# vincekurtz/quadruped_drake

Measured on NVIDIA B200. Metric: whole-body QP control steps/sec, higher is better.
Workload: dtype f64

## Files before the change

### quadruped_drake_b200/csrc/wbc_device.cuh

```cuda
#pragma once
#include <stdint.h>
#include <math.h>
#include <stddef.h>
#include <type_traits>
#include "wbc.h"

#ifndef WBC_DEV
#define WBC_DEV __device__ __forceinline__
#endif
#ifndef WBC_FULL
#define WBC_FULL 0xffffffffu
#endif

namespace wbc {

constexpr int NF = 13;
constexpr int YS = 15;
constexpr int YROWS = 32;
constexpr int AR = 6;
constexpr int AC = 32;
constexpr double RANKDEF_SINVOL = 2e-3;

struct Derived {
  double clf_p[3][3];
// ... 341 lines not shown
    s.vf[leg][j] = comp(vfoot, j);
  }
  if (lane == 0 && !BIAS_ONLY) {
    s.task[7] = R0.c0.x; s.task[8] = R0.c0.y; s.task[9] = R0.c0.z;
    s.task[10] = R0.c1.x; s.task[11] = R0.c1.y; s.task[12] = R0.c1.z;
    s.task[13] = R0.c2.x; s.task[14] = R0.c2.y; s.task[15] = R0.c2.z;
  }
  __syncwarp();
}

#ifdef __CUDACC__
__device__ __noinline__
#else
static
#endif
void dynamics_pc_pass(WarpSmem& s, const wbc_model& md, int lane, int& status, const double* vel_int, double* bias_out, bool bias,
                      double* taug_out = nullptr) {
  dynamics_phase<DYN_PC>(s, md, lane, status, taug_out, vel_int, bias_out, bias);
}

struct BodyTask { double rpy[3], rpyd[3]; double N[3][3]; };
WBC_DEV void body_task(const WarpSmem& s, int lane, int& status, BodyTask& t) {
  const double r00 = s.task[7], r10 = s.task[8], r20 = s.task[9], r21 = s.task[12], r22 = s.task[15];
  const double cp = sqrt(r00 * r00 + r10 * r10);
  const int m = lane % 3;
  double num = m == 0 ? r21 : (m == 1 ? -r20 : r10);
  double den = m == 0 ? r22 : (m == 1 ? cp : r00);
  double ang = atan2(num, den);
  t.rpy[0] = shfl(ang, 0); t.rpy[1] = shfl(ang, 1); t.rpy[2] = shfl(ang, 2);
  double cy, sy;
  const double icp = cp < 1e-6 ? 0.0 : frcp(cp);
  if (cp < 1e-6) { status |= WBC_ST_GIMBAL; cy = 1.0; sy = 0.0; }
  else { cy = r00 * icp; sy = r10 * icp; }
  const double sp = -r20;
  t.N[0][0] = cy * cp; t.N[0][1] = -sy; t.N[0][2] = 0.0;
  t.N[1][0] = sy * cp; t.N[1][1] = cy;  t.N[1][2] = 0.0;
  t.N[2][0] = -sp;     t.N[2][1] = 0.0; t.N[2][2] = 1.0;
  const double wx = s.v[0], wy = s.v[1], wz = s.v[2];
  t.rpyd[0] = (cy * wx + sy * wy) * icp;
  t.rpyd[1] = -sy * wx + cy * wy;
  t.rpyd[2] = wz + sp * t.rpyd[0];
}

WBC_DEV double skew_ent(V3 r, int i, int c) {
  if (i == c) return 0.0;
  const double m = comp(r, 3 - i - c);
  return ((i + 1) % 3 == c) ? -m : m;
}
WBC_DEV int stance_slot(unsigned cmask, int k) {
  return ((cmask >> k) & 1) ? __popc(cmask & ((1u << k) - 1)) : -1;
}
WBC_DEV int stance_foot(unsigned cmask, int slot) {
  int k = 0, cnt = 0;
#pragma unroll
  for (int kk = 0; kk < 4; ++kk) { if ((cmask >> kk) & 1) { if (cnt == slot) k = kk; ++cnt; } }
  return k;
}

WBC_DEV void build_base_system(WarpSmem& s, int lane, unsigned cmask, double kd, int& status) {
  bool bad = false;
  if (lane < 12) {
    const int k = lane / 3, i = lane % 3;
    if ((cmask >> k) & 1) {
      const int i1 = (i + 1) % 3, i2 = (i + 2) % 3;
      const V3 ci = mk(s.L[k][0][i], s.L[k][1][i], s.L[k][2][i]);
      const V3 c1 = mk(s.L[k][0][i1], s.L[k][1][i1], s.L[k][2][i1]);
      const V3 c2 = mk(s.L[k][0][i2], s.L[k][1][i2], s.L[k][2][i2]);
      const V3 cx = cross(c1, c2);
      const double det = dot(ci, cx);
      const double vol2 = dot(ci, ci) * dot(c1, c1) * dot(c2, c2);
      bad = !(det * det > RANKDEF_SINVOL * RANKDEF_SINVOL * vol2);
      const V3 li = frcp(bad ? 1.0 : det) * cx;
      const V3 rh = ld3(s.rho[k]);
      const V3 lxr = cross(rh, li);
      s.AK[k][i][0] = lxr.x; s.AK[k][i][1] = lxr.y; s.AK[k][i][2] = lxr.z;
      s.AK[k][i][3] = li.x; s.AK[k][i][4] = li.y; s.AK[k][i][5] = li.z;
      const V3 r = mk(-s.Jdv[k][0] - kd * s.vf[k][0], -s.Jdv[k][1] - kd * s.vf[k][1], -s.Jdv[k][2] - kd * s.vf[k][2]);
      s.AK[k][i][6] = dot(li, r);
    }
  }
  if (__any_sync(WBC_FULL, bad)) status |= WBC_ST_RANKDEF;
  __syncwarp();
  const int c = lane;
  double col[AR];
#pragma unroll
  for (int r = 0; r < AR; ++r) col[r] = 0.0;
  if (c < 6 || c == 31) {
    const int cc = c < 6 ? c : 6;
#pragma unroll
    for (int r = 0; r < 6; ++r) col[r] = c < 6 ? s.Mb[c][r] : -s.hb[r];
#pragma unroll
    for (int k = 0; k < 4; ++k) {
      if (!((cmask >> k) & 1)) continue;
#pragma unroll
      for (int a = 0; a < 3; ++a) {
        const double ak = s.AK[k][a][cc];
#pragma unroll
        for (int r = 0; r < 6; ++r) col[r] = fma(-s.Mb[6 + 3 * k + a][r], ak, col[r]);
      }
    }
  } else if (c < 18) {
    const int k = (c - 6) / 3, i = (c - 6) % 3;
    if ((cmask >> k) & 1) {
      const V3 rh = ld3(s.rho[k]);
#pragma unroll
      for (int r = 0; r < 3; ++r) { col[r] = skew_ent(rh, i, r); col[3 + r] = (r == i) ? -1.0 : 0.0; }
    } else {
#pragma unroll
      for (int r = 0; r < 6; ++r) col[r] = s.Mb[c][r];
    }
  }
#pragma unroll
  for (int r = 0; r < AR; ++r) s.A[r][c] = col[r];
  __syncwarp();
}

WBC_DEV unsigned gauss_jordan(WarpSmem& s, int lane, int m, int n, int& status, unsigned long long& rowmap) {
  unsigned used = 0;
  rowmap = 0ull;
  for (int r = 0; r < m; ++r) {
    const double arc0 = s.A[r][lane];
    const bool eligible = lane < n && !((used >> lane) & 1);
    int pcol;
    const double best = warp_max_lane(eligible ? fabs(arc0) : 0.0, pcol);
    if (!(best > 1e-9)) {
      status |= WBC_ST_RANKDEF;
      continue;
    }
    const double piv = shfl(arc0, pcol);
    const double arc = arc0 * frcp(piv);
    if (lane != pcol) {
#pragma unroll
      for (int i = 0; i < AR; ++i) {
        if (i < m) {
          const double f = s.A[i][pcol];
          s.A[i][lane] = fma(-f, arc, s.A[i][lane]);
        }
      }
      s.A[r][lane] = arc;
    }
    rowmap |= (unsigned long long)(r + 1) << (3 * pcol);
    used |= 1u << pcol;
    __syncwarp();
  }
  return used;
}

WBC_DEV double zent(const WarpSmem& s, int lane, int var, unsigned long long rowmap) {
  const int r = (int)((rowmap >> (3 * var)) & 7ull) - 1;
  const double a = s.A[r >= 0 ? r : 0][lane];
  return r >= 0 ? (lane == 31 ? a : -a) : (var == lane ? 1.0 : 0.0);
}

struct TriPairs { int i[3], k[3]; };
template <int N> WBC_DEV TriPairs tri_pairs(int lane) {
  TriPairs t;
#pragma unroll
  for (int h = 0; h < 3; ++h) {
    const int e = lane + 32 * h;
    int ii = 0;
#pragma unroll
    for (int c = 1; c < N; ++c) ii += (c * (c + 1) / 2 <= e) ? 1 : 0;
    t.i[h] = e < N * (N + 1) / 2 ? ii : -1;
    t.k[h] = e - ii * (ii + 1) / 2;
  }
  return t;
}

template <int N, class SM> WBC_DEV void reduced_hessian(SM& s, int lane, int nf, bool tau_rows, bool extra, const TriPairs& tp) {
  s.y[lane] = s.cw[lane] * (s.Y[lane][NF] - s.ct[lane]);
  const double wb = s.cw[0], wl0 = s.cw[6], wl1 = s.cw[9], wl2 = s.cw[12], wl3 = s.cw[15];
#pragma unroll
  for (int h = 0; h < 3; ++h) {
    const int i = tp.i[h], k = tp.k[h];
    if (i < 0) continue;
    const double* yi = &s.Y[0][i];
    const double* yk = &s.Y[0][k];
    auto term = [&](int r) { return yi[r * YS] * yk[r * YS]; };
    auto leg = [&](int r) { return fma(yi[(r + 2) * YS], yk[(r + 2) * YS], fma(yi[(r + 1) * YS], yk[(r + 1) * YS], term(r))); };
    const double b0 = fma(yi[2 * YS], yk[2 * YS], fma(yi[1 * YS], yk[1 * YS], term(0)));
    const double b1 = fma(yi[5 * YS], yk[5 * YS], fma(yi[4 * YS], yk[4 * YS], term(3)));
    double acc = wb * (b0 + b1);
    acc = fma(wl0, leg(6), acc); acc = fma(wl1, leg(9), acc); acc = fma(wl2, leg(12), acc); acc = fma(wl3, leg(15), acc);
    if (tau_rows) {
      double t0 = 0.0, t1 = 0.0;
#pragma unroll
      for (int r = 18; r < 30; r += 2) { t0 = fma(yi[r * YS], yk[r * YS], t0); t1 = fma(yi[(r + 1) * YS], yk[(r + 1) * YS], t1); }
      acc = fma(s.cw[18], t0 + t1, acc);
    }
    if (extra) acc = fma(s.cw[30] * yi[30 * YS], yk[30 * YS], fma(s.cw[31] * yi[31 * YS], yk[31 * YS], acc));
    if (i >= nf) acc = (i == k) ? 1.0 : 0.0;
    s.H[i][k] = acc;
  }
  __syncwarp();
}

template <int N, class SM> WBC_DEV void cholesky_factor(SM& s, int lane, int& status, const TriPairs& tp) {
  for (int j = 0; j < N; ++j) {
    const double dj = s.H[j][j];
    if (!(dj > 1e-300)) { status |= WBC_ST_NOTPD; }
    const double rd = frcp(dj > 1e-300 ? dj : 1.0);
#pragma unroll
    for (int h = 0; h < 3; ++h) {
      const int i = tp.i[h], k = tp.k[h];
      if (i >= 0 && k > j) s.H[i][k] = fma(-s.H[i][j] * rd, s.H[k][j], s.H[i][k]);
    }
    __syncwarp();
  }
  if (lane < N) { const double dk = s.H[lane][lane]; s.d[lane] = frsqrt(dk > 1e-300 ? dk : 1.0); }
  __syncwarp();
#pragma unroll
  for (int h = 0; h < 3; ++h) {
    const int i = tp.i[h], k = tp.k[h];
    if (i >= 0) s.H[i][k] *= s.d[k];
  }
  __syncwarp();
}
struct Ineq { int ra, rb; double ca, cb, bound; };
struct IneqSet {
  unsigned cmask; double mu; int nfric; int nextra; int ntl; const double* effort;
  double extra_bound[2];
};
WBC_DEV Ineq get_ineq(const IneqSet& S, int i) {
  Ineq q; q.ra = q.rb = 0; q.ca = q.cb = 0.0; q.bound = 0.0;
  if (i < S.nfric) {
    int sl = i >> 2, t = i & 3, k = 0, cnt = 0;
#pragma unroll
    for (int kk = 0; kk < 4; ++kk) { if ((S.cmask >> kk) & 1) { if (cnt == sl) k = kk; ++cnt; } }
    q.ra = 6 + 3 * k + (t >> 1); q.ca = (t & 1) ? -1.0 : 1.0;
    q.rb = 6 + 3 * k + 2; q.cb = -S.mu; q.bound = 0.0;
  } else if (i < S.nfric + S.nextra) {
    const int e = i - S.nfric;
    q.ra = 30 + e; q.ca = 1.0; q.bound = S.extra_bound[e];
  } else {
    const int e = i - S.nfric - S.nextra;
    const int k = e % 12;
    q.ra = 18 + k; q.ca = e < 12 ? 1.0 : -1.0; q.bound = S.effort[k];
  }
  return q;
}

template <int N, class SM> WBC_DEV double tri_fwd_lane(const SM& s, int lane, double rhs) {
  const bool row = lane < N;
  const int li = row ? lane : N - 1;
  const double dinv = s.d[li];
  double acc = row ? rhs : 0.0, bl = 0.0;
#pragma unroll
  for (int j = 0; j < N; ++j) {
    const double bj = shfl(acc * dinv, j);
    if (lane == j) bl = bj;
    else if (lane > j) acc = fma(-s.H[li][j], bj, acc);
  }
  return bl;
}
template <int N, class SM> WBC_DEV double tri_bwd_lane(const SM& s, int lane, double rhs) {
  const bool row = lane < N;
  const int li = row ? lane : N - 1;
  const double dinv = s.d[li];
  double acc = row ? rhs : 0.0, xl = 0.0;
#pragma unroll
  for (int j = N - 1; j >= 0; --j) {
    const double xj = shfl(acc * dinv, j);
    if (lane == j) xl = xj;
    else if (lane < j) acc = fma(-s.H[j][li], xj, acc);
  }
  return xl;
}

template <int N, class SM> WBC_DEV int gi_solve_ws(SM& s, int lane, const IneqSet& S, int max_iter, int& status, int& q_out,
                                                  double& minslack, const double* Yg) {
  const int mi = S.nfric + S.nextra + S.ntl;
  const bool row = lane < N;
  const int li = row ? lane : N - 1;
  const Ineq c0 = get_ineq(S, lane < mi ? lane : 0);
  const bool have0 = lane < mi;
  double* Wl = &s.Y[lane][0];
  double yl;
  {
    double w[N];
#pragma unroll
    for (int k = 0; k < N; ++k) {
      double acc = Wl[k];
#pragma unroll
      for (int j = 0; j < k; ++j) acc = fma(-w[j], s.H[k][j], acc);
      w[k] = acc * s.d[k];
    }
#pragma unroll
    for (int k = 0; k < N; ++k) Wl[k] = w[k];
    __syncwarp();
    {
      const double* wc = &s.Y[0][li];
      double b0 = 0.0, b1 = 0.0;
#pragma unroll
      for (int r = 0; r < 18; r += 2) { b0 = fma(wc[r * YS], s.y[r], b0); b1 = fma(wc[(r + 1) * YS], s.y[r + 1], b1); }
      if (s.cw[18] != 0.0) {
#pragma unroll
        for (int r = 18; r < 30; r += 2) { b0 = fma(wc[r * YS], s.y[r], b0); b1 = fma(wc[(r + 1) * YS], s.y[r + 1], b1); }
      }
      b0 = fma(wc[30 * YS], s.y[30], b0); b1 = fma(wc[31 * YS], s.y[31], b1);
      if (row) s.dm[lane] = b0 + b1;
    }
    __syncwarp();
    double ya = Wl[NF], ya1 = 0.0;
#pragma unroll
    for (int k = 0; k < N; ++k) { if (k & 1) ya1 = fma(-w[k], s.dm[k], ya1); else ya = fma(-w[k], s.dm[k], ya); }
    yl = ya + ya1;
    __syncwarp();
    s.y[lane] = yl;
  }
  __syncwarp();
  double ddl0 = 0.0, ddl1 = 0.0;
  {
    const double* wa = &s.Y[c0.ra][0];
    const double* wb = &s.Y[c0.rb][0];
#pragma unroll
    for (int k = 0; k < N; ++k) { const double t = fma(c0.ca, wa[k], c0.cb * wb[k]); ddl0 = fma(t, t, ddl0); }
    if (mi > 32) {
      const Ineq c1 = get_ineq(S, lane + 32 < mi ? lane + 32 : 0);
      const double* va = &s.Y[c1.ra][0];
      const double* vb = &s.Y[c1.rb][0];
#pragma unroll
      for (int k = 0; k < N; ++k) { const double t = fma(c1.ca, va[k], c1.cb * vb[k]); ddl1 = fma(t, t, ddl1); }
    }
  }
  double* const Ril = ri_rows(s) + li * NF;
  {
    double* r0 = ri_rows(s);
    for (int e = lane; e < NF * NF; e += 32) r0[e] = 0.0;
  }
  __syncwarp();
  int q = 0, iters = 0;
  unsigned long long activemask = 0ull;
  double ul = 0.0;
  int actl = 0;
  minslack = 0.0;
  double violl = 0.0;
  auto select = [&](bool& any, int& p_out, int& wl) {
    double viol = 0.0; int who = lane;
    if (have0 && !((activemask >> lane) & 1ull)) {
      const double ta = c0.ca * s.y[c0.ra], tb = c0.cb * s.y[c0.rb];
      const double sl = c0.bound - ta - tb;
      if (sl < -1e-10 * (1.0 + fabs(c0.bound) + fabs(ta) + fabs(tb))) viol = -sl;
    }
    if (mi > 32) {
      const Ineq c1 = get_ineq(S, lane + 32 < mi ? lane + 32 : 0);
      if (lane + 32 < mi && !((activemask >> (lane + 32)) & 1ull)) {
        const double ta = c1.ca * s.y[c1.ra], tb = c1.cb * s.y[c1.rb];
        const double sl = c1.bound - ta - tb;
        if (sl < -1e-10 * (1.0 + fabs(c1.bound) + fabs(ta) + fabs(tb)) && -sl > viol) { viol = -sl; who = lane + 32; }
      }
    }
    violl = viol;
    wl = warp_argmax_hi(viol, any);
    p_out = (mi > 32) ? shfl(who, wl) : wl;
  };
  bool any; int p, wlane;
  select(any, p, wlane);
  for (;;) {
    if (!any) break;
    Ineq cp;
    if (p < 32) {
      const int rr = shfl(c0.ra | (c0.rb << 8), p);
      cp.ra = rr & 0xff; cp.rb = rr >> 8;
      cp.ca = shfl(c0.ca, p); cp.cb = shfl(c0.cb, p); cp.bound = shfl(c0.bound, p);
    } else {
      cp = get_ineq(S, p);
    }
    const double nca = -cp.ca, ncb = -cp.cb;
    double up = 0.0;
    bool fail = false;
    const double dd = (p < 32) ? shfl(ddl0, p & 31) : shfl(ddl1, p & 31);
    for (;;) {
      if (++iters > max_iter) { status |= WBC_ST_MAXITER; fail = true; break; }
      const double dself = fma(nca, s.Y[cp.ra][li], ncb * s.Y[cp.rb][li]);
      if (row) s.dm[lane] = dself;
      __syncwarp();
      double zn = 0.0, zn1 = 0.0, wd = 0.0, wd1 = 0.0;
      switch (q) {
#define WBC_ACC(K)                                                                                   \
        case K:                                                                                      \
          if (K < N) {                                                                               \
            const double dk_ = s.dm[K < N ? K : 0];                                                  \
            if (K & 1) { zn1 = fma(dk_, dk_, zn1); wd1 = fma(Wl[K < N ? K : 0], dk_, wd1); }         \
            else { zn = fma(dk_, dk_, zn); wd = fma(Wl[K < N ? K : 0], dk_, wd); }                   \
          }
        WBC_ACC(0) WBC_ACC(1) WBC_ACC(2) WBC_ACC(3) WBC_ACC(4) WBC_ACC(5) WBC_ACC(6) WBC_ACC(7) WBC_ACC(8) WBC_ACC(9) WBC_ACC(10)
        WBC_ACC(11) WBC_ACC(12)
#undef WBC_ACC
        default: break;
      }
      double rk = 0.0, rk1 = 0.0;
      switch (q) {
#define WBC_RI(K)                                                                                    \
        case K + 1:                                                                                  \
          if (K < N) {                                                                               \
            if (K & 1) rk1 = fma(Ril[K < N ? K : 0], s.dm[K < N ? K : 0], rk1);                      \
            else rk = fma(Ril[K < N ? K : 0], s.dm[K < N ? K : 0], rk);                              \
          }
        WBC_RI(12) WBC_RI(11) WBC_RI(10) WBC_RI(9) WBC_RI(8) WBC_RI(7) WBC_RI(6) WBC_RI(5) WBC_RI(4) WBC_RI(3) WBC_RI(2) WBC_RI(1)
        WBC_RI(0)
#undef WBC_RI
        default: break;
      }
      zn += zn1; wd += wd1; rk += rk1;
      const int qc = q < N ? q : N - 1;
      const double dq = s.dm[qc], wq = Wl[qc];
      const double sp = cp.bound - cp.ca * s.y[cp.ra] - cp.cb * s.y[cp.rb];
      const bool zok = zn > 1e-14 * fmax(dd, 1e-300);
      const double zs = zok ? zn : 1.0;
      const double izn = frcp(zs);
      const double rs = frsqrt(zs);
      const double nrm = zs * rs;
      const double alpha = dq > 0.0 ? -nrm : nrm;
      const double hv = fma(-dq, alpha, zs);
      const double ihv = frcp(hv);
      int l;
      const double t1 = warp_min_lane((lane < q && rk > 0.0) ? fmax(ul * frcp(rk), 0.0) + 0.0 : INFINITY, l);
      const double t2 = zok ? -sp * izn : INFINITY;
      const double t = fmin(t1, t2);
      if (!(t < INFINITY)) { status |= WBC_ST_INFEASIBLE; fail = true; break; }
      const bool dual_only = !(t2 < INFINITY);
      if (lane < q) ul -= t * rk;
      up += t;
      __syncwarp();
      if (!dual_only) { yl = fma(t, wd, yl); s.y[lane] = yl; }
      if (!dual_only && t2 <= t1) {
        activemask |= 1ull << p;
        if (lane == 0 && q < N - 1) s.dm[qc] = dq - alpha;
        __syncwarp();
        bool nany; int np, nwl;
        select(nany, np, nwl);
        double rqq = dq, irq = dq > 0.0 ? rs : -rs;
        if (q < N - 1) {
          const double sc = (wd - alpha * wq) * ihv;
          switch (q) {
#define WBC_UPD(K) case K: if (K < N) Wl[K < N ? K : 0] = fma(-sc, s.dm[K < N ? K : 0], Wl[K < N ? K : 0]);
            WBC_UPD(0) WBC_UPD(1) WBC_UPD(2) WBC_UPD(3) WBC_UPD(4) WBC_UPD(5) WBC_UPD(6) WBC_UPD(7) WBC_UPD(8) WBC_UPD(9) WBC_UPD(10)
            WBC_UPD(11) WBC_UPD(12)
#undef WBC_UPD
            default: break;
          }
          rqq = alpha; irq = dq > 0.0 ? -rs : rs;
        }
        if (lane < q) { Rent(s, q, lane) = dself; Ril[qc] = -rk * irq; }
        if (lane == q) { Rent(s, q, q) = rqq; Ril[qc] = irq; ul = up; actl = p; }
        ++q;
        any = nany; p = np; wlane = nwl;
        __syncwarp();
        break;
      }
      {
        __syncwarp();
        const int dropped = shfl(actl, l);
        activemask &= ~(1ull << dropped);
        for (int jj = l; jj < q - 1; ++jj) { if (lane <= jj + 1) Rent(s, jj, lane) = Rent(s, jj + 1, lane); }
        if (lane <= q) Rent(s, q - 1, lane) = 0.0;
        {
          const bool mv = row && lane >= l && lane < q - 1;
          const double* src = mv ? Ril + NF : Ril;
          for (int j = 0; j < q; ++j) {
// ... 370 lines not shown
  if (in && in->v) { for (int i = lane; i < WBC_NV; i += 32) s.v[i] = in->v[i]; }
  else { for (int i = lane; i < WBC_NV; i += 32) s.v[i] = a.v[inst * WBC_NV + i]; }
  if (in && in->traj) { for (int i = lane; i < WBC_NTRAJ; i += 32) s.traj[i] = in->traj[i]; }
  else { for (int i = lane; i < WBC_NTRAJ; i += 32) async_copy8(&s.traj[i], a.traj + inst * WBC_NTRAJ + i); }
  {
    const uint8_t* cptr = (in && in->contact) ? in->contact : a.contact + inst * 4;
#pragma unroll
    for (int k = 0; k < 4; ++k) cmask |= (cptr[k] ? 1u : 0u) << k;
  }
  const int nc = __popc(cmask);
  __syncwarp();
  if (KIND == WBC_CTRL_PC) {
    WBC_CTA_MEET(1, pcs->sync_all);
    dynamics_pc_pass(s, md, lane, status, nullptr, nullptr, false, pcs->tg);
  } else dynamics_phase<DYN_STEP>(s, md, lane, status, nullptr);
  async_wait_all();
  __syncwarp();
  {
    bool nonfin = lane < WBC_NQ && !isfinite(s.q[lane]);
    nonfin |= lane < WBC_NV && !isfinite(s.v[lane]);
    nonfin |= !isfinite(s.traj[lane]) || (lane < WBC_NTRAJ - 32 && !isfinite(s.traj[32 + lane]));
    if (__any_sync(WBC_FULL, nonfin)) status |= WBC_ST_NONFINITE;
  }
  BodyTask bt;
  body_task(s, lane, status, bt);
  const int mtask = 6 + 3 * (4 - nc);
  double Vpc = 0.0, errpc = 0.0;
  bool pc_ok = true;
  if (KIND == WBC_CTRL_PC) {
    if (nc == 0) { status |= WBC_ST_UNSUPPORTED; pc_ok = false; }
    else pc_precompute(s, *pcs, md, pr, bt, lane, cmask, mtask, status, Vpc, errpc);
  }
  const int ndelta = (KIND == WBC_CTRL_CLF) ? 1 : 0;
  const int n = 18 + ndelta, m = 6;
  build_base_system(s, lane, cmask, pr.contact_damping, status);
  unsigned long long rowmap;
  const unsigned used = gauss_jordan(s, lane, m, n, status, rowmap);
  const unsigned freemask = ~used & ((n >= 32) ? 0xffffffffu : ((1u << n) - 1u));
  const int nf = __popc(freemask);
  const bool isfree = (freemask >> lane) & 1u;
  const int widx = __popc(freemask & ((1u << lane) - 1u));
  const int ycol = lane == 31 ? NF : (isfree ? widx : -1);
  constexpr int NA = (KIND == WBC_CTRL_CLF) ? NF : NF - 1;
  const bool ok = nf <= NA && pc_ok;
  double err = 0.0;
  int nextra = 0;
  double extra_bound = 0.0, Vl = 0.0, PFl = 0.0, csum = 0.0;
  if (ok) {
    {
      double* y0 = &s.Y[0][0];
#pragma unroll
      for (int e = lane; e < YROWS * YS / 2; e += 32) { y0[2 * e] = 0.0; y0[2 * e + 1] = 0.0; }
    }
    s.cw[lane] = 0.0; s.ct[lane] = 0.0;
    __syncwarp();
    build_common_rows(s, lane, ycol, cmask, rowmap, vdmap);
    const double* tr = s.traj;
    if (KIND == WBC_CTRL_ID) {
      double rdd[3], add[3];
#pragma unroll
      for (int i = 0; i < 3; ++i) {
        rdd[i] = tr[15 + i] - pr.id_kp_body_rpy * (bt.rpy[i] - tr[9 + i]) - pr.id_kd_body_rpy * (bt.rpyd[i] - tr[12 + i]);
        add[i] = tr[6 + i] - pr.id_kp_body_p * (s.q[4 + i] - tr[i]) - pr.id_kd_body_p * (s.v[3 + i] - tr[3 + i]);
        err += (bt.rpy[i] - tr[9 + i]) * (bt.rpy[i] - tr[9 + i]) + (s.q[4 + i] - tr[i]) * (s.q[4 + i] - tr[i]);
      }
      if (lane < 3) { s.cw[lane] = pr.id_w_body; s.ct[lane] = bt.N[lane][0] * rdd[0] + bt.N[lane][1] * rdd[1] + bt.N[lane][2] * rdd[2]; }
      else if (lane < 6) { s.cw[lane] = pr.id_w_body; s.ct[lane] = add[lane - 3]; }
      else if (lane < 18) {
        const int k = (lane - 6) / 3, i = (lane - 6) % 3;
        if ((cmask >> k) & 1) { s.cw[lane] = pr.reg_f; s.ct[lane] = 0.0; }
        else {
          const double pfoot = s.q[4 + i] + s.rho[k][i];
          const double as = tr[42 + 3 * k + i] - pr.id_kp_foot * (pfoot - tr[18 + 3 * k + i]) - pr.id_kd_foot * (s.vf[k][i] - tr[30 + 3 * k + i]);
          s.cw[lane] = pr.id_w_foot; s.ct[lane] = as - s.Jdv[k][i];
        }
      } else if (lane < 30) { s.cw[lane] = pr.reg_tau; s.ct[lane] = 0.0; }
#pragma unroll
      for (int k = 0; k < 4; ++k)
        if (!((cmask >> k) & 1)) {
#pragma unroll
          for (int i = 0; i < 3; ++i) { const double e = s.q[4 + i] + s.rho[k][i] - tr[18 + 3 * k + i]; err += e * e; }
        }
    }
    if (KIND == WBC_CTRL_CLF) {
      double xt = 0.0, xdt = 0.0, xddn = 0.0, jdv = 0.0, kap = 0.0;
      bool taskrow = false;
      int type = 0;
      if (lane < 3) {
        taskrow = true; type = 0;
        xt = bt.rpy[lane] - tr[9 + lane];
        xdt = s.v[lane] - (bt.N[lane][0] * tr[12] + bt.N[lane][1] * tr[13] + bt.N[lane][2] * tr[14]);
        xddn = bt.N[lane][0] * tr[15] + bt.N[lane][1] * tr[16] + bt.N[lane][2] * tr[17];
      } else if (lane < 6) {
        const int i = lane - 3;
        taskrow = true; type = 1;
        xt = s.q[4 + i] - tr[i]; xdt = s.v[3 + i] - tr[3 + i]; xddn = tr[6 + i];
      } else if (lane < 18) {
        const int k = (lane - 6) / 3, i = (lane - 6) % 3;
        if (!((cmask >> k) & 1)) {
          taskrow = true; type = 2;
          xt = s.q[4 + i] + s.rho[k][i] - tr[18 + 3 * k + i]; xdt = s.vf[k][i] - tr[30 + 3 * k + i]; xddn = tr[42 + 3 * k + i];
          jdv = s.Jdv[k][i];
        } else { s.cw[lane] = pr.reg_f; s.ct[lane] = 0.0; }
      } else if (lane < 30) { s.cw[lane] = pr.reg_tau; s.ct[lane] = 0.0; }
      if (taskrow) {
        const double p11 = dv.clf_p[type][0], p12 = dv.clf_p[type][1], p22 = dv.clf_p[type][2];
        kap = p12 * xt + p22 * xdt;
        s.cw[lane] = 1.0;
        s.ct[lane] = xddn - kap / pr.clf_r - jdv - 2.0 * kap;
        Vl = p11 * xt * xt + 2.0 * p12 * xt * xdt + p22 * xdt * xdt;
        PFl = (p11 * xt + p12 * xdt) * xdt;
        csum = kap * (jdv - xddn);
        err = xt * xt;
      }
      s.y[lane] = kap;
      Vl = warp_sum(Vl); PFl = warp_sum(PFl); csum = warp_sum(csum); err = warp_sum(err);
      __syncwarp();
      const int cdel = 18;
      if (ycol >= 0) {
        double acc = 0.0;
        for (int r = 0; r < 18; ++r) acc = fma(2.0 * s.y[r], s.Y[r][ycol], acc);
        const double isdel = (lane == cdel) ? 1.0 : 0.0;
        s.Y[30][ycol] = acc - isdel;
        s.Y[31][ycol] = isdel;
      }
      if (lane == 31) { s.cw[31] = 2.0 * pr.clf_w_delta; s.ct[31] = 0.0; }
      nextra = 1;
      extra_bound = -dv.clf_gamma[nc < 4 ? 1 : 0] * Vl - 2.0 * PFl - 2.0 * csum;
    }
    if (KIND == WBC_CTRL_PC) {
      pc_rows(s, *pcs, lane, ycol, mtask);
      if (lane < 6 || (lane < 18 && !((cmask >> ((lane - 6) / 3)) & 1))) { s.cw[lane] = 1.0; s.ct[lane] = 0.0; }
      else if (lane < 18) { s.cw[lane] = pr.reg_f; s.ct[lane] = 0.0; }
      else if (lane < 30) { s.cw[lane] = pr.reg_tau; s.ct[lane] = 0.0; }
      nextra = (a.kind == WBC_CTRL_PC) ? 1 : 0;
      extra_bound = 0.0;
      err = errpc;
    }
    __syncwarp();
  }
  c.status = status; c.cmask = cmask; c.nf = nf; c.nextra = nextra; c.ok = ok; c.pc_ok = pc_ok;
  c.extra_bound = extra_bound; c.err = err; c.Vl = Vl; c.PFl = PFl; c.csum = csum; c.Vpc = Vpc;
}

template <int KIND, class SM>
WBC_DEV void solve_instance(SM& s, const wbc_model& md, const wbc_params& pr, const StepArgs& a, long long inst, int lane,
                            const StepCarry& c, const double* vdmap = nullptr, const double* yrec = nullptr) {
  constexpr int NA = (KIND == WBC_CTRL_CLF) ? NF : NF - 1;
  int status = c.status;
  const unsigned cmask = c.cmask;
  const int nc = __popc(cmask), nf = c.nf, nextra = c.nextra;
  const double extra_bound = c.extra_bound, err = c.err, Vl = c.Vl, PFl = c.PFl, csum = c.csum, Vpc = c.Vpc;
  if (c.ok) {
    const TriPairs tp = tri_pairs<NA>(lane);
    reduced_hessian<NA>(s, lane, nf, pr.reg_tau != 0.0, KIND != WBC_CTRL_ID, tp);
    cholesky_factor<NA>(s, lane, status, tp);
    IneqSet S;
    S.cmask = cmask; S.mu = pr.mu; S.nfric = 4 * nc; S.nextra = nextra; S.ntl = pr.torque_limits ? 24 : 0;
    S.effort = md.effort; S.extra_bound[0] = extra_bound; S.extra_bound[1] = 0.0;
    int qact = 0; double minslack = 0.0;
    int iters = 0;
    if (!(status & WBC_ST_NOTPD)) {
      iters = gi_solve_ws<NA>(s, lane, S, pr.max_iter, status, qact, minslack, (SM::kVd && a.vd != nullptr) ? yrec : nullptr);
    }
    const bool want_vd = SM::kVd && a.vd && lane < 18;
    double vdv = 0.0;
    if (want_vd) {
      const double* mrow = vdmap + lane * YS;
      vdv = mrow[NF];
      for (int w = 0; w < nf; ++w) vdv = fma(mrow[w], s.x[w], vdv);
    }
    const bool nonfin = (lane < 12 && !(isfinite(s.y[18 + lane]) && isfinite(s.y[6 + lane]))) || !isfinite(vdv);
    if (__any_sync(WBC_FULL, nonfin)) status |= WBC_ST_NONFINITE;
    const bool failed = status != 0;
    const double res = minslack < 0.0 ? -minslack : 0.0;
    if (lane < 12) {
      a.tau[inst * WBC_NU + md.act_index[lane]] = failed ? 0.0 : s.y[18 + lane];
      if (a.f) a.f[inst * 12 + lane] = (!failed && ((cmask >> (lane / 3)) & 1)) ? s.y[6 + lane] : 0.0;
    }
    if (want_vd) a.vd[inst * WBC_NV + (lane < 6 ? lane : md.v_index[lane - 6])] = failed ? 0.0 : vdv;
    if (a.lam) {
      double* lrow = &s.Rp[0];
      __syncwarp();
      lrow[lane] = 0.0;
      if (lane < WBC_NLAM - 32) lrow[32 + lane] = 0.0;
      __syncwarp();
      if (!failed && lane < qact) {
        const int id = s.act[lane];
        int slot;
        if (id < S.nfric) slot = 4 * stance_foot(cmask, id >> 2) + (id & 3);
        else if (id < S.nfric + S.nextra) slot = 16 + (id - S.nfric);
        else { const int e = id - S.nfric - S.nextra; slot = 18 + md.act_index[e % 12] + (e < 12 ? 0 : 12); }
        lrow[slot] = s.u[lane];
      }
      __syncwarp();
      a.lam[inst * WBC_NLAM + lane] = lrow[lane];
      if (lane < WBC_NLAM - 32) a.lam[inst * WBC_NLAM + 32 + lane] = lrow[32 + lane];
    }
    double obj = 0.0;
    {
      const bool refrow = lane < 6 || (lane < 18 && !((cmask >> ((lane - 6) / 3)) & 1)) || (KIND == WBC_CTRL_CLF && lane == 31);
      if (refrow) { const double yy = s.y[lane], t = s.ct[lane], w = s.cw[lane]; obj = 0.5 * w * yy * yy - w * t * yy; }
    }
    obj = warp_sum(obj);
    if (lane == 0) {
      double* mt = a.metrics + inst * WBC_NMETRIC;
      double delta = 0.0;
      if (KIND == WBC_CTRL_ID) { mt[0] = 0.0; mt[1] = err; mt[2] = res; mt[3] = 0.0; }
      if (KIND == WBC_CTRL_CLF) {
        delta = s.y[31];
        mt[0] = Vl; mt[1] = err; mt[2] = res; mt[3] = 2.0 * PFl + s.y[30] + delta + 2.0 * csum;
      }
      if (KIND == WBC_CTRL_PC) {
        mt[0] = Vpc; mt[1] = err; mt[2] = res; mt[3] = s.y[30];
      }
      if (a.qp_info) { double* qi = a.qp_info + inst * 4; qi[0] = obj; qi[1] = res; qi[2] = delta; qi[3] = (double)iters; }
    }
  } else {
    if (c.pc_ok) status |= WBC_ST_RANKDEF;
    if (lane < 12) { a.tau[inst * WBC_NU + lane] = 0.0; if (a.f) a.f[inst * 12 + lane] = 0.0; }
    if (a.vd && lane < 18) a.vd[inst * WBC_NV + lane] = 0.0;
    if (a.lam) { a.lam[inst * WBC_NLAM + lane] = 0.0; if (lane < WBC_NLAM - 32) a.lam[inst * WBC_NLAM + 32 + lane] = 0.0; }
    if (lane < 4) a.metrics[inst * WBC_NMETRIC + lane] = 0.0;
    if (a.qp_info && lane < 4) a.qp_info[inst * 4 + lane] = 0.0;
  }
  if (lane == 0) a.status[inst] = status;
  __syncwarp();
}


WBC_DEV void dynamics_instance(WarpSmem& s, const wbc_model& md, const double* q, const double* v, const DynOut& o,
                               long long inst, int lane) {
  int status = 0;
  for (int i = lane; i < WBC_NQ; i += 32) s.q[i] = q[inst * WBC_NQ + i];
  for (int i = lane; i < WBC_NV; i += 32) s.v[i] = v[inst * WBC_NV + i];
  __syncwarp();
  double* taug = &s.A[0][0];
  dynamics_phase<DYN_PARITY>(s, md, lane, status, taug);
  auto didx = [&](int c) { return c < 6 ? c : md.v_index[c - 6]; };
  if (o.M) {
    double* M = o.M + inst * 324;
    for (int e = lane; e < 324; e += 32) {
      const int r = e / 18, c = e % 18;
      double val;
      if (r < 6) val = s.Mb[c][r];
      else if (c < 6) val = s.Mb[r][c];
      else if ((r - 6) / 3 == (c - 6) / 3) { const int i = (r - 6) % 3, j = (c - 6) % 3; val = s.Mleg[(r - 6) / 3][sym3(i < j ? i : j, i < j ? j : i)]; }
      else val = 0.0;
      M[didx(r) * 18 + didx(c)] = val;
    }
  }
  if (lane < 18) {
    const double cv = lane < 6 ? s.hb[lane] : s.hj[lane - 6];
    if (o.Cv) o.Cv[inst * 18 + didx(lane)] = cv;
    if (o.taug) o.taug[inst * 18 + didx(lane)] = taug[lane];
  }
  if (o.Jfeet) {
    double* J = o.Jfeet + inst * 216;
    for (int e = lane; e < 216; e += 32) {
      const int k = e / 54, i = (e % 54) / 18, c = e % 18;
      const V3 rh = ld3(s.rho[k]);
      double val = 0.0;
      if (c < 3) val = -skew_ent(rh, i, c);
      else if (c < 6) val = (c - 3 == i) ? 1.0 : 0.0;
      else if ((c - 6) / 3 == k) val = s.L[k][i][(c - 6) % 3];
      J[k * 54 + i * 18 + didx(c)] = val;
    }
  }
  if (lane < 12) {
    if (o.Jdv) o.Jdv[inst * 12 + lane] = s.Jdv[lane / 3][lane % 3];
    if (o.pfeet) o.pfeet[inst * 12 + lane] = s.q[4 + lane % 3] + s.rho[lane / 3][lane % 3];
  }
  __syncwarp();
}

WBC_DEV void coriolis_instance(WarpSmem& s, PcSmem& pc, const wbc_model& md, const double* q, const double* v, double* Cout,
                               double* Jdout, long long inst, int lane) {
  int status = 0;
  for (int i = lane; i < WBC_NQ; i += 32) s.q[i] = q[inst * WBC_NQ + i];
  for (int i = lane; i < WBC_NV; i += 32) s.v[i] = v[inst * WBC_NV + i];
  __syncwarp();
  dynamics_phase<DYN_STEP_JD>(s, md, lane, status, nullptr);
  auto didx = [&](int c) { return c < 6 ? c : md.v_index[c - 6]; };
  if (lane < 18) pc.vi[lane] = lane < 6 ? s.v[lane] : s.v[md.v_index[lane - 6]];
  __syncwarp();
  dynamics_phase<DYN_BIAS>(s, md, lane, status, nullptr, pc.vi, pc.tg);
  if (Cout) {
    for (int j = 0; j < 18; ++j) {
      if (lane < 18) { pc.w[lane] = (lane == j) ? 1.0 : 0.0; pc.vw[lane] = pc.vi[lane] + ((lane == j) ? 1.0 : 0.0); }
      __syncwarp();
      dynamics_phase<DYN_BIAS>(s, md, lane, status, nullptr, pc.vw, pc.bvw);
      dynamics_phase<DYN_BIAS>(s, md, lane, status, nullptr, pc.w, pc.bw);
      if (lane < 18) Cout[inst * 324 + didx(lane) * 18 + didx(j)] = 0.5 * (pc.bvw[lane] - pc.tg[lane] - pc.bw[lane]);
      __syncwarp();
    }
  }
  if (Jdout) {
    double* J = Jdout + inst * 216;
    for (int e = lane; e < 216; e += 32) {
      const int k = e / 54, i = (e % 54) / 18, c = e % 18;
      const V3 dv = mk(s.vf[k][0] - s.v[3], s.vf[k][1] - s.v[4], s.vf[k][2] - s.v[5]);
      double val = 0.0;
      if (c < 3) val = -skew_ent(dv, i, c);
      else if (c >= 6 && (c - 6) / 3 == k) val = s.Ld[k][i][(c - 6) % 3];
      J[k * 54 + i * 18 + didx(c)] = val;
    }
  }
  __syncwarp();
}
// ... 37 lines not shown
```

Measured before the change: 44.92 million.

## Build reduced Hessian with FP64 MMA and factor Cholesky in registers

Replaces the shared-memory triangular Hessian build with FP64 m8n8k4 mma.sync tiles that compute Y^T W Y, with the linear term folded in as an extra column. The Cholesky factorization then runs on the register-resident fragments using shuffles instead of per-column shared-memory updates and __syncwarp calls. It also drops the separate pass that computed dm by reusing that fused column. This cuts shared-memory traffic and warp syncs, at the cost of many more shuffles and a layout-heavy register scheme that could raise register pressure.

```diff
diff --git a/quadruped_drake_b200/csrc/wbc_device.cuh b/quadruped_drake_b200/csrc/wbc_device.cuh
--- a/quadruped_drake_b200/csrc/wbc_device.cuh
+++ b/quadruped_drake_b200/csrc/wbc_device.cuh
@@ -517,67 +517,94 @@
   return r >= 0 ? (lane == 31 ? a : -a) : (var == lane ? 1.0 : 0.0);
 }
 
-struct TriPairs { int i[3], k[3]; };
-template <int N> WBC_DEV TriPairs tri_pairs(int lane) {
-  TriPairs t;
-#pragma unroll
-  for (int h = 0; h < 3; ++h) {
-    const int e = lane + 32 * h;
-    int ii = 0;
-#pragma unroll
-    for (int c = 1; c < N; ++c) ii += (c * (c + 1) / 2 <= e) ? 1 : 0;
-    t.i[h] = e < N * (N + 1) / 2 ? ii : -1;
-    t.k[h] = e - ii * (ii + 1) / 2;
-  }
-  return t;
-}
-
-template <int N, class SM> WBC_DEV void reduced_hessian(SM& s, int lane, int nf, bool tau_rows, bool extra, const TriPairs& tp) {
-  s.y[lane] = s.cw[lane] * (s.Y[lane][NF] - s.ct[lane]);
-  const double wb = s.cw[0], wl0 = s.cw[6], wl1 = s.cw[9], wl2 = s.cw[12], wl3 = s.cw[15];
-#pragma unroll
-  for (int h = 0; h < 3; ++h) {
-    const int i = tp.i[h], k = tp.k[h];
-    if (i < 0) continue;
-    const double* yi = &s.Y[0][i];
-    const double* yk = &s.Y[0][k];
-    auto term = [&](int r) { return yi[r * YS] * yk[r * YS]; };
-    auto leg = [&](int r) { return fma(yi[(r + 2) * YS], yk[(r + 2) * YS], fma(yi[(r + 1) * YS], yk[(r + 1) * YS], term(r))); };
-    const double b0 = fma(yi[2 * YS], yk[2 * YS], fma(yi[1 * YS], yk[1 * YS], term(0)));
-    const double b1 = fma(yi[5 * YS], yk[5 * YS], fma(yi[4 * YS], yk[4 * YS], term(3)));
-    double acc = wb * (b0 + b1);
-    acc = fma(wl0, leg(6), acc); acc = fma(wl1, leg(9), acc); acc = fma(wl2, leg(12), acc); acc = fma(wl3, leg(15), acc);
-    if (tau_rows) {
-      double t0 = 0.0, t1 = 0.0;
-#pragma unroll
-      for (int r = 18; r < 30; r += 2) { t0 = fma(yi[r * YS], yk[r * YS], t0); t1 = fma(yi[(r + 1) * YS], yk[(r + 1) * YS], t1); }
-      acc = fma(s.cw[18], t0 + t1, acc);
-    }
-    if (extra) acc = fma(s.cw[30] * yi[30 * YS], yk[30 * YS], fma(s.cw[31] * yi[31 * YS], yk[31 * YS], acc));
-    if (i >= nf) acc = (i == k) ? 1.0 : 0.0;
-    s.H[i][k] = acc;
-  }
-  __syncwarp();
-}
-
-template <int N, class SM> WBC_DEV void cholesky_factor(SM& s, int lane, int& status, const TriPairs& tp) {
+#ifdef __CUDA_ARCH__
+WBC_DEV void dmma_8x8x4(double& d0, double& d1, double a, double b, int lane) {
+  (void)lane;
+  asm("mma.sync.aligned.m8n8k4.row.col.f64.f64.f64.f64 {%0, %1}, {%2}, {%3}, {%0, %1};" : "+d"(d0), "+d"(d1) : "d"(a), "d"(b));
+}
+#else
+WBC_DEV void dmma_8x8x4(double& d0, double& d1, double a, double b, int lane) {
+  const int g = lane >> 2, n = 2 * (lane & 3);
+  for (int k = 0; k < 4; ++k) {
+    const double ak = __shfl_sync(WBC_FULL, a, 4 * g + k);
+    const double b0 = __shfl_sync(WBC_FULL, b, 4 * n + k), b1 = __shfl_sync(WBC_FULL, b, 4 * n + 4 + k);
+    d0 = fma(ak, b0, d0);
+    d1 = fma(ak, b1, d1);
+  }
+}
+#endif
+
+template <int N, class SM> WBC_DEV void hessian_cholesky(SM& s, int lane, int nf, bool tau_rows, bool extra, int& status) {
+  const int g = lane >> 2, c = lane & 3;
+  constexpr int GB = NF - 8;
+  double h[4][2] = {{0.0, 0.0}, {0.0, 0.0}, {0.0, 0.0}, {0.0, 0.0}};
+#pragma unroll
+  for (int kb = 0; kb < YROWS / 4; ++kb) {
+    if ((kb == 5 || kb == 6) && !tau_rows) continue;
+    if (kb == 7 && !tau_rows && !extra) continue;
+    const int r = 4 * kb + c;
+    const bool on = r < 18 || (r < 30 ? tau_rows : extra);
+    const double w = on ? s.cw[r] : 0.0;
+    const double y0 = (on && g < nf) ? s.Y[r][g] : 0.0;
+    const double y1 = (on && 8 + g < nf) ? s.Y[r][8 + g < nf ? 8 + g : 0] : 0.0;
+    const double a1 = g == GB ? (on ? s.Y[r][NF] - s.ct[r] : 0.0) : y1;
+    const double b0 = w * y0, b1 = w * y1;
+    dmma_8x8x4(h[0][0], h[0][1], y0, b0, lane);
+    dmma_8x8x4(h[2][0], h[2][1], a1, b0, lane);
+    dmma_8x8x4(h[3][0], h[3][1], a1, b1, lane);
+  }
+#pragma unroll
+  for (int t = 0; t < 4; ++t) {
+#pragma unroll
+    for (int e = 0; e < 2; ++e) {
+      const int i = 8 * (t >> 1) + g, k = 8 * (t & 1) + 2 * c + e;
+      if (t != 1 && ((i >= nf && i != NF) || k >= nf)) h[t][e] = (i == k) ? 1.0 : 0.0;
+    }
+  }
+#pragma unroll
   for (int j = 0; j < N; ++j) {
-    const double dj = s.H[j][j];
+    const int K = j >> 3, e = j & 1, cj = (j & 7) >> 1;
+    const double dj = shfl(h[3 * K][e], 4 * (j & 7) + cj);
     if (!(dj > 1e-300)) { status |= WBC_ST_NOTPD; }
     const double rd = frcp(dj > 1e-300 ? dj : 1.0);
-#pragma unroll
-    for (int h = 0; h < 3; ++h) {
-      const int i = tp.i[h], k = tp.k[h];
-      if (i >= 0 && k > j) s.H[i][k] = fma(-s.H[i][j] * rd, s.H[k][j], s.H[i][k]);
-    }
-    __syncwarp();
-  }
-  if (lane < N) { const double dk = s.H[lane][lane]; s.d[lane] = frsqrt(dk > 1e-300 ? dk : 1.0); }
-  __syncwarp();
-#pragma unroll
-  for (int h = 0; h < 3; ++h) {
-    const int i = tp.i[h], k = tp.k[h];
-    if (i >= 0) s.H[i][k] *= s.d[k];
+    double ck[2][2];
+#pragma unroll
+    for (int Kc = (j < 7 ? 0 : 1); Kc < 2; ++Kc)
+#pragma unroll
+      for (int ee = 0; ee < 2; ++ee) ck[Kc][ee] = shfl(h[2 * Kc + K][e], 4 * (2 * c + ee) + cj);
+#pragma unroll
+    for (int I = (j < 7 ? 0 : 1); I < 2; ++I) {
+      const int i = 8 * I + g;
+      const double fi = -shfl(h[2 * I + K][e], 4 * g + cj) * rd;
+      if (i > j) {
+#pragma unroll
+        for (int Kc = (j < 7 ? 0 : 1); Kc <= I; ++Kc) {
+#pragma unroll
+          for (int ee = 0; ee < 2; ++ee) {
+            const int k = 8 * Kc + 2 * c + ee;
+            if (k > j) h[2 * I + Kc][ee] = fma(fi, ck[Kc][ee], h[2 * I + Kc][ee]);
+          }
+        }
+      }
+    }
+  }
+#pragma unroll
+  for (int I = 0; I < 2; ++I) {
+#pragma unroll
+    for (int e = 0; e < 2; ++e) {
+      const int k = 8 * I + g;
+      if (g == 2 * c + e && k < N) { const double dk = h[3 * I][e]; s.d[k] = frsqrt(dk > 1e-300 ? dk : 1.0); }
+    }
+  }
+  __syncwarp();
+#pragma unroll
+  for (int t = 0; t < 4; ++t) {
+#pragma unroll
+    for (int e = 0; e < 2; ++e) {
+      const int i = 8 * (t >> 1) + g, k = 8 * (t & 1) + 2 * c + e;
+      if (t != 1 && k <= i && i < N) s.H[i][k] = h[t][e] * s.d[k];
+      if (t >= 2 && g == GB && k < N) s.dm[k] = h[t][e] * s.d[k];
+    }
   }
   __syncwarp();
 }
@@ -652,25 +679,10 @@
     }
 #pragma unroll
     for (int k = 0; k < N; ++k) Wl[k] = w[k];
-    __syncwarp();
-    {
-      const double* wc = &s.Y[0][li];
-      double b0 = 0.0, b1 = 0.0;
-#pragma unroll
-      for (int r = 0; r < 18; r += 2) { b0 = fma(wc[r * YS], s.y[r], b0); b1 = fma(wc[(r + 1) * YS], s.y[r + 1], b1); }
-      if (s.cw[18] != 0.0) {
-#pragma unroll
-        for (int r = 18; r < 30; r += 2) { b0 = fma(wc[r * YS], s.y[r], b0); b1 = fma(wc[(r + 1) * YS], s.y[r + 1], b1); }
-      }
-      b0 = fma(wc[30 * YS], s.y[30], b0); b1 = fma(wc[31 * YS], s.y[31], b1);
-      if (row) s.dm[lane] = b0 + b1;
-    }
-    __syncwarp();
     double ya = Wl[NF], ya1 = 0.0;
 #pragma unroll
     for (int k = 0; k < N; ++k) { if (k & 1) ya1 = fma(-w[k], s.dm[k], ya1); else ya = fma(-w[k], s.dm[k], ya); }
     yl = ya + ya1;
-    __syncwarp();
     s.y[lane] = yl;
   }
   __syncwarp();
@@ -1347,9 +1359,7 @@
   const int nc = __popc(cmask), nf = c.nf, nextra = c.nextra;
   const double extra_bound = c.extra_bound, err = c.err, Vl = c.Vl, PFl = c.PFl, csum = c.csum, Vpc = c.Vpc;
   if (c.ok) {
-    const TriPairs tp = tri_pairs<NA>(lane);
-    reduced_hessian<NA>(s, lane, nf, pr.reg_tau != 0.0, KIND != WBC_CTRL_ID, tp);
-    cholesky_factor<NA>(s, lane, status, tp);
+    hessian_cholesky<NA>(s, lane, nf, pr.reg_tau != 0.0, KIND != WBC_CTRL_ID, status);
     IneqSet S;
     S.cmask = cmask; S.mu = pr.mu; S.nfric = 4 * nc; S.nextra = nextra; S.ntl = pr.torque_limits ? 24 : 0;
     S.effort = md.effort; S.extra_bound[0] = extra_bound; S.extra_bound[1] = 0.0;
```

After: 46.17 million, median of 6. +2.8%, better.
